# showlab/EgoVLP

Measured on AMD Instinct MI355X. Metric: clip-pairs/sec (whole node), 4f/224^2 ViT-B + 32-tok text, B=32/GPU, train step (fwd+gather+EgoNCE+bwd+AdamW), higher is better.
Workload: dtype fp16 (every Linear and both attentions of the video blocks, forward and backward) + bf16 (patch embedding, text tower, heads) MFMA operands, fp32 accumulate

## Files before the change

### egovlp_amd/csrc/gemm_nt.hip

```cpp
#include "common.h"
#include "egovlp_hip.h"

namespace {

constexpr int BM = 128, BN = 128, BK = 32;
constexpr int PLANE_BYTES = BM * BK * 2;

struct Frag4 {
  bf16x8_t v[4];
};

__device__ __forceinline__ int swz_g(int x) { return (0x78 >> (2 * x)) & 3; }

__device__ __forceinline__ void glds16(const void* g, char* lds_wave_base) {
  __builtin_amdgcn_global_load_lds((const __attribute__((address_space(1))) void*)g,
                                   (__attribute__((address_space(3))) void*)lds_wave_base, 16, 0, 0);
}

__device__ __forceinline__ void nt_epilogue4(const egv_gemm_desc& p, f32x4_t v, int m, int n) {
  if (p.alpha != 1.0f) v *= p.alpha;
  if (p.bias) v += *(const f32x4_t*)(p.bias + n);
  if (p.act == EGV_ACT_GELU) {
    if (p.aux_out) *(f32x4_t*)(p.aux_out + (long)m * p.ldaux + n) = v;
#pragma unroll
    for (int e = 0; e < 4; ++e) v[e] = gelu_f(v[e]);
  } else if (p.act == EGV_ACT_GELU_BWD) {
    const f32x4_t zv = *(const f32x4_t*)(p.aux_in + (long)m * p.ldaux + n);
#pragma unroll
    for (int e = 0; e < 4; ++e) v[e] *= gelu_grad_f(zv[e]);
  } else if (p.act == EGV_ACT_RELU_BWD) {
    const f32x4_t zv = *(const f32x4_t*)(p.aux_in + (long)m * p.ldaux + n);
#pragma unroll
    for (int e = 0; e < 4; ++e) v[e] = zv[e] > 0.f ? v[e] : 0.f;
  }
  if (p.residual) v += *(const f32x4_t*)(p.residual + (long)m * p.ldr + n);
  if (p.out_f32) *(f32x4_t*)(p.out_f32 + (long)m * p.ldo + n) = v;
  if (p.out_hi) {
    bf16_t h[4], l[4];
#pragma unroll
    for (int e = 0; e < 4; ++e) split_bf16(v[e], h[e], l[e]);
    *(u32x2_t*)(p.out_hi + (long)m * p.ldoh + n) = (u32x2_t){pack2(h[0], h[1]), pack2(h[2], h[3])};
    if (p.out_lo) *(u32x2_t*)(p.out_lo + (long)m * p.ldoh + n) = (u32x2_t){pack2(l[0], l[1]), pack2(l[2], l[3])};
  }
}

template <int PASSES>
__global__ __launch_bounds__(256, 2) void gemm_nt_kernel(const egv_gemm_desc p) {
  extern __shared__ __attribute__((aligned(16))) char smem[];
  constexpr int NPL = (PASSES == 3) ? 4 : 2;
  constexpr int STAGE_BYTES = NPL * PLANE_BYTES;

  const int tid = threadIdx.x;
  const int lane = tid & 63;
  const int wave = __builtin_amdgcn_readfirstlane(tid >> 6);
  const int wm = wave >> 1, wn = wave & 1;

  const int tiles_n = (p.N + BN - 1) / BN;
  const int tiles_m = (p.M + BM - 1) / BM;
  const int nwg = tiles_m * tiles_n;
  const int wg = xcd_remap(blockIdx.x, nwg);
  const int tm = wg / tiles_n, tn = wg % tiles_n;
  const int m0 = tm * BM, n0 = tn * BN;

  const int ksplit = p.ksplit > 1 ? p.ksplit : 1;
  const int z = blockIdx.y;
  const int ksteps_total = p.K / BK;
  const int ksteps_per = (ksteps_total + ksplit - 1) / ksplit;
  const int ks_begin = z * ksteps_per;
  const int ks_end = min(ksteps_total, ks_begin + ksteps_per);
  const int nk = ks_end - ks_begin;

  const int srcchunk = (lane & 3) ^ swz_g((lane >> 4) & 3);
  const bf16_t* asrc[2][2];
  const bf16_t* bsrc[2][2];
#pragma unroll
  for (int q = 0; q < 2; ++q) {
    const int row = (wave * 2 + q) * 16 + (lane >> 2);
    const long ar = min(m0 + row, p.M - 1);
    const long br = min(n0 + row, p.N - 1);
    const long koff = (long)ks_begin * BK + srcchunk * 8;
    asrc[0][q] = p.a_hi + ar * p.lda + koff;
    bsrc[0][q] = p.b_hi + br * p.ldb + koff;
    if (PASSES == 3) {
      asrc[1][q] = p.a_lo + ar * p.lda + koff;
      bsrc[1][q] = p.b_lo + br * p.ldb + koff;
    }
  }

  auto stage = [&](int buf) {
    char* base = smem + buf * STAGE_BYTES + wave * 2048;
#pragma unroll
    for (int q = 0; q < 2; ++q) {
      glds16(asrc[0][q], base + 0 * PLANE_BYTES + q * 1024);
      glds16(bsrc[0][q], base + (NPL / 2) * PLANE_BYTES + q * 1024);
      if (PASSES == 3) {
        glds16(asrc[1][q], base + 1 * PLANE_BYTES + q * 1024);
        glds16(bsrc[1][q], base + 3 * PLANE_BYTES + q * 1024);
      }
      asrc[0][q] += BK;
      bsrc[0][q] += BK;
      if (PASSES == 3) {
        asrc[1][q] += BK;
        bsrc[1][q] += BK;
      }
    }
  };

  const int frow = lane & 15;
  const int foff = frow * 64 + (((lane >> 4) ^ swz_g(frow >> 2)) * 16);
  const int a_off = (wm * 64) * 64 + foff;
  const int b_off = (wn * 64) * 64 + foff;

  f32x4_t acc[4][4];
#pragma unroll
  for (int i = 0; i < 4; ++i)
#pragma unroll
    for (int j = 0; j < 4; ++j) acc[i][j] = (f32x4_t){0.f, 0.f, 0.f, 0.f};

  if (nk > 0) stage(0);
  for (int t = 0; t < nk; ++t) {
    __syncthreads();
    if (t + 1 < nk) stage((t + 1) & 1);
    const char* sb = smem + (t & 1) * STAGE_BYTES;
    Frag4 ah, bh, al, bl;
#pragma unroll
    for (int f = 0; f < 4; ++f) {
      ah.v[f] = *(const bf16x8_t*)(sb + 0 * PLANE_BYTES + a_off + f * 16 * 64);
      bh.v[f] = *(const bf16x8_t*)(sb + (NPL / 2) * PLANE_BYTES + b_off + f * 16 * 64);
      if (PASSES == 3) {
        al.v[f] = *(const bf16x8_t*)(sb + 1 * PLANE_BYTES + a_off + f * 16 * 64);
        bl.v[f] = *(const bf16x8_t*)(sb + 3 * PLANE_BYTES + b_off + f * 16 * 64);
      }
    }
#pragma unroll
    for (int i = 0; i < 4; ++i)
#pragma unroll
      for (int j = 0; j < 4; ++j) {
        if (PASSES == 3) {
          acc[i][j] = __builtin_amdgcn_mfma_f32_16x16x32_bf16(bl.v[j], ah.v[i], acc[i][j], 0, 0, 0);
          acc[i][j] = __builtin_amdgcn_mfma_f32_16x16x32_bf16(bh.v[j], al.v[i], acc[i][j], 0, 0, 0);
        }
        acc[i][j] = __builtin_amdgcn_mfma_f32_16x16x32_bf16(bh.v[j], ah.v[i], acc[i][j], 0, 0, 0);
      }
  }

  const int lm = lane & 15;
  const int ln = (lane >> 4) * 4;
#pragma unroll
  for (int i = 0; i < 4; ++i) {
    const int m = m0 + wm * 64 + i * 16 + lm;
    if (m >= p.M) continue;
#pragma unroll
    for (int j = 0; j < 4; ++j) {
      const int n = n0 + wn * 64 + j * 16 + ln;
      if (n >= p.N) continue;
      f32x4_t v = acc[i][j];
      if (ksplit > 1) {
        *(f32x4_t*)(p.partial + ((long)z * p.M + m) * p.N + n) = v;
        continue;
      }
      nt_epilogue4(p, v, m, n);
    }
  }
}

__global__ __launch_bounds__(256) void splitk_reduce_kernel(const float* __restrict__ partial, float* __restrict__ out,
                                                            long mn, int ksplit, int accumulate,
                                                            const float* __restrict__ partial2, float* __restrict__ out2,
                                                            long n2, int blocks1) {
  if ((int)blockIdx.x >= blocks1) {
    partial = partial2;
    out = out2;
    mn = n2;
    accumulate = 0;
  }
  const long i4 = ((long)((int)blockIdx.x >= blocks1 ? (int)blockIdx.x - blocks1 : (int)blockIdx.x) * blockDim.x + threadIdx.x) * 4;
  if (i4 >= mn) return;
  f32x4_t s = egv_load<EGV_NT_REDUCE_LD, f32x4_t>(partial + i4);
  for (int z = 1; z < ksplit; ++z) s += egv_load<EGV_NT_REDUCE_LD, f32x4_t>(partial + (long)z * mn + i4);
  if (accumulate) s += *(const f32x4_t*)(out + i4);
  egv_store<EGV_NT_WGRAD>(out + i4, s);
}

constexpr int RED_MAX_T = 8;
struct ReduceTable {
  const float* partial[RED_MAX_T];
  float* out[RED_MAX_T];
  float* colsum[RED_MAX_T];
  long mn[RED_MAX_T];
  int m[RED_MAX_T], ks[RED_MAX_T];
  int blk_start[RED_MAX_T + 1];
  int blocks1[RED_MAX_T];
  int count;
};
__global__ __launch_bounds__(256) void splitk_reduce_multi_kernel(const ReduceTable t) {
  int e = 0;
  while (e + 1 < t.count && (int)blockIdx.x >= t.blk_start[e + 1]) ++e;
  const int local = (int)blockIdx.x - t.blk_start[e];
  const int ks = t.ks[e];
  const float* partial = t.partial[e];
  float* out = t.out[e];
  long mn = t.mn[e];
  long i4;
  if (local >= t.blocks1[e]) {
    partial += (long)ks * mn;
    out = t.colsum[e];
    mn = t.m[e];
    i4 = ((long)(local - t.blocks1[e]) * 256 + threadIdx.x) * 4;
  } else {
    i4 = ((long)local * 256 + threadIdx.x) * 4;
  }
  if (i4 >= mn) return;
  f32x4_t s = egv_load<EGV_NT_REDUCE_LD, f32x4_t>(partial + i4);
  for (int z = 1; z < ks; ++z) s += egv_load<EGV_NT_REDUCE_LD, f32x4_t>(partial + (long)z * mn + i4);
  egv_store<EGV_NT_WGRAD>(out + i4, s);
}

}

extern "C" int egv_splitk_reduce_multi(int32_t count, const float* const* partial, float* const* out, const int64_t* mn, const int32_t* ksplit,
                                       float* const* colsum, const int32_t* m, void* stream) {
  if (count < 1 || count > RED_MAX_T || !partial || !out || !mn || !ksplit) return EGV_ERR_ARG;
  ReduceTable t = {};
  int nb = 0;
  for (int i = 0; i < count; ++i) {
    if (!partial[i] || !out[i] || mn[i] <= 0 || mn[i] % 4 != 0 || ksplit[i] < 2) return EGV_ERR_ARG;
    const bool cs = colsum && colsum[i];
    if (cs && (!m || m[i] <= 0 || m[i] % 4 != 0)) return EGV_ERR_ARG;
    t.partial[i] = partial[i]; t.out[i] = out[i]; t.colsum[i] = cs ? colsum[i] : nullptr;
    t.mn[i] = mn[i]; t.m[i] = cs ? m[i] : 0; t.ks[i] = ksplit[i];
    t.blk_start[i] = nb;
    t.blocks1[i] = (int)((mn[i] / 4 + 255) / 256);
    nb += t.blocks1[i] + (cs ? (m[i] / 4 + 255) / 256 : 0);
  }
  t.blk_start[count] = nb;
  t.count = count;
  EGV_LAUNCH(splitk_reduce_multi_kernel, dim3(nb), dim3(256), 0, (hipStream_t)stream, t);
  EGV_CHECK_LAUNCH();
  return EGV_OK;
}

int egv_gemm_big_launch(const egv_gemm_desc& p, hipStream_t s, int variant);
bool egv_gemm_big_supports(const egv_gemm_desc& p);

__global__ __launch_bounds__(256) void splitk_reduce_epilogue_kernel(const egv_gemm_desc p, int ksplit) {
  const long i4 = ((long)blockIdx.x * blockDim.x + threadIdx.x) * 4;
  const long mn = (long)p.M * p.N;
  if (i4 >= mn) return;
  f32x4_t s = *(const f32x4_t*)(p.partial + i4);
  for (int z = 1; z < ksplit; ++z) s += *(const f32x4_t*)(p.partial + (long)z * mn + i4);
  const int m = (int)(i4 / p.N), n = (int)(i4 - (long)m * p.N);
  nt_epilogue4(p, s, m, n);
}

static int gemm_variant(const egv_gemm_desc& p) {
  const bool big_ok = egv_gemm_big_supports(p);
  if (p.trans) return big_ok ? 3 : -1;
  if (p.passes == 2 || p.passes == 4) return big_ok ? 3 : -1;
  const long big_tiles = (long)((p.M + 255) / 256) * ((p.N + 255) / 256) * (p.ksplit > 1 ? p.ksplit : 1);
  if (big_ok && big_tiles >= 128) return 3;
  return 1;
}

extern "C" int egv_gemm_nt(const egv_gemm_desc* d, void* stream) {
  const egv_gemm_desc& p = *d;
  if (!p.a_hi || !p.b_hi) return EGV_ERR_ARG;
  if (p.passes < 1 || p.passes > 4) return EGV_ERR_ARG;
  if ((p.passes == 2 || p.passes == 3) && (!p.a_lo || !p.b_lo)) return EGV_ERR_ARG;
  if (p.out_fmt < 0 || p.out_fmt > 4) return EGV_ERR_ARG;
  if (p.M <= 0 || p.N <= 0 || p.K <= 0) return EGV_ERR_ARG;
  if (p.N % 4 != 0 || p.lda % 8 != 0 || p.ldb % 8 != 0) return EGV_ERR_ARG;
  if (!p.trans && p.K % BK != 0) return EGV_ERR_ARG;
  if (p.ksplit > 1 && !p.partial) return EGV_ERR_ARG;
  if (p.colsum && !p.trans) return EGV_ERR_ARG;
  if (p.grid_cap != 0 && (p.grid_cap < 8 || p.grid_cap > 256 || p.grid_cap % 8 != 0)) return EGV_ERR_ARG;
  const int variant = gemm_variant(p);
  if (variant < 0) return EGV_ERR_ARG;
  if (p.aux_bf16 < 0 || p.aux_bf16 > 3) return EGV_ERR_ARG;
  if (p.aux_bf16 && (variant < 3 || p.act == EGV_ACT_RELU_BWD)) return EGV_ERR_ARG;
  if (p.aux_bf16 == 3 && p.passes != 4 && p.passes != 2) return EGV_ERR_ARG;
  if ((p.passes == 2 || p.passes == 4 || p.out_fmt != 0) && (variant < 3 || (p.passes != 2 && p.passes != 4))) return EGV_ERR_ARG;
  if ((p.passes == 2 || p.out_fmt != 0) && (p.trans || p.ksplit > 1)) return EGV_ERR_ARG;
  if (p.passes == 4 && !p.trans && p.ksplit > 1) return EGV_ERR_ARG;
  if (p.alpha != 1.0f && p.trans && !(p.alpha > 0.f)) return EGV_ERR_ARG;
  const int tiles = ((p.M + BM - 1) / BM) * ((p.N + BN - 1) / BN);
  const int ks = p.ksplit > 1 ? p.ksplit : 1;
  dim3 grid(tiles, ks), block(256);
  hipStream_t s = (hipStream_t)stream;
  if (variant >= 3) {
    const int rc = egv_gemm_big_launch(p, s, variant);
    if (rc) return rc;
  } else if (p.passes == 3) {
    EGV_LAUNCH(gemm_nt_kernel<3>, grid, block, 2 * 4 * PLANE_BYTES, s, p);
  } else {
    EGV_LAUNCH(gemm_nt_kernel<1>, grid, block, 2 * 2 * PLANE_BYTES, s, p);
  }
  EGV_CHECK_LAUNCH();
  if (ks > 1 && !p.trans && variant < 3) {
    if (p.accumulate) return EGV_ERR_ARG;
    const long mn4 = (long)p.M * p.N / 4;
    EGV_LAUNCH(splitk_reduce_epilogue_kernel, dim3((int)((mn4 + 255) / 256)), dim3(256), 0, s, p, ks);
    EGV_CHECK_LAUNCH();
  } else if (ks > 1 && p.accumulate == 2) {
    if (!p.trans || !p.out_f32 || p.ldo != p.N) return EGV_ERR_ARG;
  } else if (ks > 1) {
    if (!p.out_f32 || p.ldo != p.N) return EGV_ERR_ARG;
    const long mn = (long)p.M * p.N;
    const int blocks = (int)((mn / 4 + 255) / 256);
    if (p.colsum && p.M % 4 != 0) return EGV_ERR_ARG;
    const int blocks2 = p.colsum ? (p.M / 4 + 255) / 256 : 0;
    EGV_LAUNCH(splitk_reduce_kernel, dim3(blocks + blocks2), dim3(256), 0, s, p.partial, p.out_f32, mn, ks, p.accumulate,
               p.partial + (long)ks * mn, p.colsum, (long)p.M, blocks);
    EGV_CHECK_LAUNCH();
  }
  return EGV_OK;
}
```

### egovlp_amd/csrc/text_layer.hip

```cpp
#include <hip/hip_runtime.h>

#include "layer_call.h"

namespace {

bool geom_ok(const egv_text_geom& g) {
  if (g.B <= 0 || g.L <= 0 || g.H <= 0 || g.D != g.H * 64 || g.Hd <= 0 || g.D % 32 || g.Hd % 32) return false;
  if ((g.fwd_passes != 1 && g.fwd_passes != 3) || (g.bwd_passes != 1 && g.bwd_passes != 3) || g.bwd_passes > g.fwd_passes) return false;
  if (!(g.attn_p >= 0.0f && g.attn_p < 1.0f) || !(g.ffn_p >= 0.0f && g.ffn_p < 1.0f)) return false;
  for (int i = 0; i < 4; ++i)
    if (g.nt_ksplit_fwd[i] < 1 || g.nt_ksplit_bwd[i] < 1 || g.wgrad_ksplit[i] < 1) return false;
  return true;
}

void wshape(const egv_text_geom& g, int i, int64_t& N, int64_t& K) {
  switch (i) {
    case 0: N = 3 * (int64_t)g.D; K = g.D; break;
    case 1: N = g.D; K = g.D; break;
    case 2: N = g.Hd; K = g.D; break;
    default: N = g.D; K = g.Hd; break;
  }
}

struct FwdLayout {
  int64_t x_hi, x_lo, qkv, c_hi, c_lo, lse, s1, sa_hi, sa_lo, sa, mean1, rstd1, h_hi, h_lo, z, s2raw, s2, mean2, rstd2, partial;
  int64_t total;
};

FwdLayout fwd_layout(const egv_text_geom& g) {
  const int64_t M = (int64_t)g.B * g.L, D = g.D, Hd = g.Hd;
  const bool lo = g.fwd_passes == 3;
  FwdLayout L;
  Bump b;
  auto plane = [&](int64_t cols) { return b.take(M * cols * 2); };
  auto plane_lo = [&](int64_t cols) { return lo ? b.take(M * cols * 2) : (int64_t)-1; };
  L.x_hi = plane(D); L.x_lo = plane_lo(D);
  L.qkv = b.take(M * 3 * D * 4);
  L.c_hi = plane(D); L.c_lo = plane_lo(D);
  L.lse = b.take((int64_t)g.B * g.H * g.L * 4);
  L.s1 = b.take(M * D * 4);
  L.sa_hi = plane(D); L.sa_lo = plane_lo(D);
  L.sa = b.take(M * D * 4);
  L.mean1 = b.take(M * 4); L.rstd1 = b.take(M * 4);
  L.h_hi = plane(Hd); L.h_lo = plane_lo(Hd);
  L.z = g.train ? b.take(M * Hd * 4) : (int64_t)-1;
  L.s2raw = g.ffn_p > 0.0f ? b.take(M * D * 4) : (int64_t)-1;
  L.s2 = b.take(M * D * 4);
  L.mean2 = b.take(M * 4); L.rstd2 = b.take(M * 4);
  int64_t pmax = 0;
  for (int i = 0; i < 4; ++i) {
    int64_t N, K;
    wshape(g, i, N, K);
    if (g.nt_ksplit_fwd[i] > 1) pmax = pmax > g.nt_ksplit_fwd[i] * M * N * 4 ? pmax : g.nt_ksplit_fwd[i] * M * N * 4;
  }
  L.partial = pmax ? b.take(pmax) : (int64_t)-1;
  L.total = b.off;
  return L;
}

struct BwdLayout {
  int64_t d_s2, g_in, g_hi, g_lo, dz_hi, dz_lo, d_sa, d_s1, ds1_hi, ds1_lo, d_ctx, dqkv, dqkv_hi, dqkv_lo, ln_work, attn_work, partial;
  int64_t total;
};

int64_t bwd_nt_cols(const egv_text_geom& g, int i) { return i == 0 ? g.Hd : g.D; }

BwdLayout bwd_layout(const egv_text_geom& g) {
  const int64_t M = (int64_t)g.B * g.L, D = g.D, Hd = g.Hd;
  const bool lo = g.bwd_passes == 3;
  BwdLayout L;
  Bump b;
  auto plane = [&](int64_t cols) { return b.take(M * cols * 2); };
  auto plane_lo = [&](int64_t cols) { return lo ? b.take(M * cols * 2) : (int64_t)-1; };
  L.d_s2 = b.take(M * D * 4);
  L.g_in = g.ffn_p > 0.0f ? b.take(M * D * 4) : (int64_t)-1;
  L.g_hi = plane(D); L.g_lo = plane_lo(D);
  L.dz_hi = plane(Hd); L.dz_lo = plane_lo(Hd);
  L.d_sa = b.take(M * D * 4);
  L.d_s1 = b.take(M * D * 4);
  L.ds1_hi = plane(D); L.ds1_lo = plane_lo(D);
  L.d_ctx = b.take(M * D * 4);
  L.dqkv = b.take(M * 3 * D * 4);
  L.dqkv_hi = plane(3 * D); L.dqkv_lo = plane_lo(3 * D);
  L.ln_work = b.take(2 * D * (int64_t)egv_layernorm_bwd_parts((int32_t)M) * 4);
  L.attn_work = b.take((int64_t)g.B * g.H * g.L * 4);
  int64_t pmax = 0;
  for (int i = 0; i < 4; ++i) {
    if (g.nt_ksplit_bwd[i] > 1) {
      const int64_t by = g.nt_ksplit_bwd[i] * M * bwd_nt_cols(g, i) * 4;
      pmax = pmax > by ? pmax : by;
    }
    int64_t N, K;
    wshape(g, i, N, K);
    if (g.wgrad_ksplit[i] > 1) {
      const int64_t by = (int64_t)g.wgrad_ksplit[i] * (N * K + N) * 4;
      pmax = pmax > by ? pmax : by;
    }
  }
  L.partial = pmax ? b.take(pmax) : (int64_t)-1;
  L.total = b.off;
  return L;
}

void grad_layout(const egv_text_geom& g, int64_t off[12], int64_t& total) {
  int64_t p = 0;
  auto take = [&](int64_t n) { const int64_t q = p; p += n; return q; };
  for (int i = 0; i < 4; ++i) { int64_t N, K; wshape(g, i, N, K); off[i] = take(N * K); }
  for (int i = 0; i < 4; ++i) { int64_t N, K; wshape(g, i, N, K); off[4 + i] = take(N); }
  for (int i = 0; i < 4; ++i) off[8 + i] = take(g.D);
  total = p;
}

}

extern "C" int64_t egv_text_layer_fwd_arena_bytes(const egv_text_geom* g) { return (g && geom_ok(*g)) ? fwd_layout(*g).total : -1; }
extern "C" int64_t egv_text_layer_bwd_arena_bytes(const egv_text_geom* g) { return (g && geom_ok(*g)) ? bwd_layout(*g).total : -1; }

extern "C" int egv_text_layer_grad_layout(const egv_text_geom* g, int64_t* offsets12, int64_t* total_floats) {
  if (!g || !geom_ok(*g) || !offsets12 || !total_floats) return EGV_ERR_ARG;
  grad_layout(*g, offsets12, *total_floats);
  return EGV_OK;
}

extern "C" int egv_text_layer_fwd(const egv_text_geom* gp, const egv_text_params* pp, const float* x, const int64_t* mask, float* out,
                                  void* arena, void* stream) {
  if (!gp || !pp || !x || !mask || !out || !arena || !geom_ok(*gp)) return EGV_ERR_ARG;
  const egv_text_geom& g = *gp;
  const egv_text_params& p = *pp;
  const FwdLayout L = fwd_layout(g);
  const int P = g.fwd_passes;
  const int32_t M = g.B * g.L, D = g.D, Hd = g.Hd;
  for (int i = 0; i < 4; ++i)
    if (!p.w_hi[i] || (P == 3 && !p.w_lo[i])) return EGV_ERR_ARG;
  char* A = (char*)arena;
  egv_bf16 *x_hi = at<egv_bf16>(A, L.x_hi), *x_lo = at<egv_bf16>(A, L.x_lo);
  egv_bf16 *c_hi = at<egv_bf16>(A, L.c_hi), *c_lo = at<egv_bf16>(A, L.c_lo);
  egv_bf16 *sa_hi = at<egv_bf16>(A, L.sa_hi), *sa_lo = at<egv_bf16>(A, L.sa_lo);
  egv_bf16 *h_hi = at<egv_bf16>(A, L.h_hi), *h_lo = at<egv_bf16>(A, L.h_lo);
  float *qkv = at<float>(A, L.qkv), *s1 = at<float>(A, L.s1), *sa = at<float>(A, L.sa), *s2 = at<float>(A, L.s2);
  float* part = at<float>(A, L.partial);

  EGV_TRY(egv_split_f32(x, D, M, D, x_hi, x_lo, D, nullptr, nullptr, 0, nullptr, stream));
  {
    egv_gemm_desc d = nt_desc(x_hi, x_lo, D, p.w_hi[0], p.w_lo[0], p.ldw[0], M, 3 * D, D, P, g.grid_cap, g.nt_ksplit_fwd[0], part);
    d.bias = p.bias[0]; d.out_f32 = qkv; d.ldo = 3 * D;
    EGV_TRY(egv_gemm_nt(&d, stream));
  }
  EGV_TRY(egv_text_attn_fwd(qkv, qkv + D, qkv + 2 * D, 3 * D, mask, g.B, g.L, g.H, P, g.attn_p, g.attn_seed, g.seed_dev, c_hi, c_lo,
                            at<float>(A, L.lse), stream));
  {
    egv_gemm_desc d = nt_desc(c_hi, c_lo, D, p.w_hi[1], p.w_lo[1], p.ldw[1], M, D, D, P, g.grid_cap, g.nt_ksplit_fwd[1], part);
    d.bias = p.bias[1]; d.residual = x; d.ldr = D; d.out_f32 = s1; d.ldo = D;
    EGV_TRY(egv_gemm_nt(&d, stream));
  }
  EGV_TRY(egv_layernorm_fwd(s1, nullptr, D, p.ln1w, p.ln1b, g.eps, M, D, nullptr, sa_hi, sa_lo, sa, D, at<float>(A, L.mean1),
                            at<float>(A, L.rstd1), stream));
  {
    egv_gemm_desc d = nt_desc(sa_hi, sa_lo, D, p.w_hi[2], p.w_lo[2], p.ldw[2], M, Hd, D, P, g.grid_cap, g.nt_ksplit_fwd[2], part);
    d.bias = p.bias[2]; d.act = EGV_ACT_GELU; d.out_hi = h_hi; d.out_lo = h_lo; d.ldoh = Hd;
    if (g.train) { d.aux_out = at<float>(A, L.z); d.ldaux = Hd; }
    EGV_TRY(egv_gemm_nt(&d, stream));
  }
  {
    egv_gemm_desc d = nt_desc(h_hi, h_lo, Hd, p.w_hi[3], p.w_lo[3], p.ldw[3], M, D, Hd, P, g.grid_cap, g.nt_ksplit_fwd[3], part);
    d.bias = p.bias[3];
    if (g.ffn_p > 0.0f) {
      float* raw = at<float>(A, L.s2raw);
      d.out_f32 = raw; d.ldo = D;
      EGV_TRY(egv_gemm_nt(&d, stream));
      EGV_TRY(egv_dropout(raw, sa, s2, (int64_t)M * D, g.ffn_p, g.ffn_seed, g.seed_dev, stream));
    } else {
      d.residual = sa; d.ldr = D; d.out_f32 = s2; d.ldo = D;
      EGV_TRY(egv_gemm_nt(&d, stream));
    }
  }
  return egv_layernorm_fwd(s2, nullptr, D, p.ln2w, p.ln2b, g.eps, M, D, nullptr, nullptr, nullptr, out, D, at<float>(A, L.mean2),
                           at<float>(A, L.rstd2), stream);
}

extern "C" int egv_text_layer_bwd(const egv_text_geom* gp, const egv_text_params* pp, const float* g_out, const int64_t* mask,
                                  const void* fwd_arena, void* bwd_arena, float* d_x, float* grads, void* stream) {
  if (!gp || !pp || !g_out || !mask || !fwd_arena || !bwd_arena || !d_x || !grads || !geom_ok(*gp) || !gp->train) return EGV_ERR_ARG;
  const egv_text_geom& g = *gp;
  const egv_text_params& p = *pp;
  const FwdLayout F = fwd_layout(g);
  const BwdLayout L = bwd_layout(g);
  int64_t goff[12], gtot;
  grad_layout(g, goff, gtot);
  const int Pb = g.bwd_passes;
  const int32_t M = g.B * g.L, D = g.D, Hd = g.Hd;
  for (int i = 0; i < 4; ++i)
    if (!p.wt_hi[i] || (Pb == 3 && !p.wt_lo[i])) return EGV_ERR_ARG;
  const char* FA = (const char*)fwd_arena;
  char* A = (char*)bwd_arena;
  const egv_bf16 *x_hi, *x_lo, *c_hi, *c_lo, *sa_hi, *sa_lo, *h_hi, *h_lo;
  saved_planes(FA, Pb, F.x_hi, F.x_lo, x_hi, x_lo);
  saved_planes(FA, Pb, F.c_hi, F.c_lo, c_hi, c_lo);
  saved_planes(FA, Pb, F.sa_hi, F.sa_lo, sa_hi, sa_lo);
  saved_planes(FA, Pb, F.h_hi, F.h_lo, h_hi, h_lo);
  const float *qkv = at<float>(FA, F.qkv), *s1 = at<float>(FA, F.s1), *s2 = at<float>(FA, F.s2);
  float* part = at<float>(A, L.partial);
  float* ln_work = at<float>(A, L.ln_work);

  auto wgrad = [&](int i, const egv_bf16* dy_hi, const egv_bf16* dy_lo, int64_t lddy, const egv_bf16* a_hi, const egv_bf16* a_lo,
                   int64_t lda) -> int {
    int64_t N, K;
    wshape(g, i, N, K);
    const egv_gemm_desc d = tn_desc(dy_hi, dy_lo, lddy, a_hi, a_lo, lda, N, K, M, Pb, grads + goff[i], grads + goff[4 + i], g.wgrad_ksplit[i],
                                    part, g.grid_cap);
    return egv_gemm_nt(&d, stream);
  };

  float* d_s2 = at<float>(A, L.d_s2);
  EGV_TRY(egv_layernorm_bwd(g_out, nullptr, nullptr, D, s2, D, p.ln2w, at<float>(FA, F.mean2), at<float>(FA, F.rstd2), M, D, nullptr, nullptr,
                            d_s2, D, nullptr, nullptr, grads + goff[10], grads + goff[11], ln_work, stream));
  const float* g_in = d_s2;
  if (g.ffn_p > 0.0f) {
    float* gi = at<float>(A, L.g_in);
    EGV_TRY(egv_dropout(d_s2, nullptr, gi, (int64_t)M * D, g.ffn_p, g.ffn_seed, g.seed_dev, stream));
    g_in = gi;
  }
  egv_bf16 *g_hi = at<egv_bf16>(A, L.g_hi), *g_lo = at<egv_bf16>(A, L.g_lo);
  EGV_TRY(egv_split_f32(g_in, D, M, D, g_hi, g_lo, D, nullptr, nullptr, 0, nullptr, stream));
  egv_bf16 *dz_hi = at<egv_bf16>(A, L.dz_hi), *dz_lo = at<egv_bf16>(A, L.dz_lo);
  {
    egv_gemm_desc d = nt_desc(g_hi, g_lo, D, p.wt_hi[3], p.wt_lo[3], p.ldwt[3], M, Hd, D, Pb, g.grid_cap, g.nt_ksplit_bwd[0], part);
    d.act = EGV_ACT_GELU_BWD; d.aux_in = at<float>(FA, F.z); d.ldaux = Hd;
    d.out_hi = dz_hi; d.out_lo = dz_lo; d.ldoh = Hd;
    EGV_TRY(egv_gemm_nt(&d, stream));
  }
  EGV_TRY(wgrad(3, g_hi, g_lo, D, h_hi, h_lo, Hd));
  EGV_TRY(wgrad(2, dz_hi, dz_lo, Hd, sa_hi, sa_lo, D));
  float* d_sa = at<float>(A, L.d_sa);
  {
    egv_gemm_desc d = nt_desc(dz_hi, dz_lo, Hd, p.wt_hi[2], p.wt_lo[2], p.ldwt[2], M, D, Hd, Pb, g.grid_cap, g.nt_ksplit_bwd[1], part);
    d.residual = d_s2; d.ldr = D; d.out_f32 = d_sa; d.ldo = D;
    EGV_TRY(egv_gemm_nt(&d, stream));
  }
  float* d_s1 = at<float>(A, L.d_s1);
  EGV_TRY(egv_layernorm_bwd(d_sa, nullptr, nullptr, D, s1, D, p.ln1w, at<float>(FA, F.mean1), at<float>(FA, F.rstd1), M, D, nullptr, nullptr,
                            d_s1, D, nullptr, nullptr, grads + goff[8], grads + goff[9], ln_work, stream));
  egv_bf16 *ds1_hi = at<egv_bf16>(A, L.ds1_hi), *ds1_lo = at<egv_bf16>(A, L.ds1_lo);
  EGV_TRY(egv_split_f32(d_s1, D, M, D, ds1_hi, ds1_lo, D, nullptr, nullptr, 0, nullptr, stream));
  EGV_TRY(wgrad(1, ds1_hi, ds1_lo, D, c_hi, c_lo, D));
  float* d_ctx = at<float>(A, L.d_ctx);
  {
    egv_gemm_desc d = nt_desc(ds1_hi, ds1_lo, D, p.wt_hi[1], p.wt_lo[1], p.ldwt[1], M, D, D, Pb, g.grid_cap, g.nt_ksplit_bwd[2], part);
    d.out_f32 = d_ctx; d.ldo = D;
    EGV_TRY(egv_gemm_nt(&d, stream));
  }
  float* dqkv = at<float>(A, L.dqkv);
  EGV_TRY(egv_text_attn_bwd(qkv, qkv + D, qkv + 2 * D, 3 * D, mask, d_ctx, at<float>(FA, F.lse), g.B, g.L, g.H, Pb, g.attn_p, g.attn_seed,
                            g.seed_dev, dqkv, dqkv + D, dqkv + 2 * D, 3 * D, at<float>(A, L.attn_work), stream));
  egv_bf16 *dq_hi = at<egv_bf16>(A, L.dqkv_hi), *dq_lo = at<egv_bf16>(A, L.dqkv_lo);
  EGV_TRY(egv_split_f32(dqkv, 3 * D, M, 3 * D, dq_hi, dq_lo, 3 * D, nullptr, nullptr, 0, nullptr, stream));
  EGV_TRY(wgrad(0, dq_hi, dq_lo, 3 * D, x_hi, x_lo, D));
  {
    egv_gemm_desc d = nt_desc(dq_hi, dq_lo, 3 * D, p.wt_hi[0], p.wt_lo[0], p.ldwt[0], M, D, 3 * D, Pb, g.grid_cap, g.nt_ksplit_bwd[3], part);
    d.residual = d_s1; d.ldr = D; d.out_f32 = d_x; d.ldo = D;
    EGV_TRY(egv_gemm_nt(&d, stream));
  }
  return EGV_OK;
}
```

Before: 1014.

## Add multi-stage LDS ring pipeline for small GEMMs and fuse text-bwd splits into layernorm

Adds a new small-tile NT GEMM kernel that uses a 4-stage LDS ring with direct global-to-LDS loads, fine-grained vmcnt waits and double-buffered register fragments. It is enabled by default through an environment toggle and replaces the two-stage kernel used by non-big GEMMs, aiming to hide global load latency. The text-layer backward also has the layernorm-backward write the bf16 hi/lo splits directly, which removes separate split kernels. Behind a compile flag, it can batch the split-k weight-gradient reductions into one multi-reduce launch. The deeper ring uses much more LDS per block (launch bounds allow 2 blocks), which may lower occupancy.

```diff
diff --git a/egovlp_amd/csrc/gemm_nt.hip b/egovlp_amd/csrc/gemm_nt.hip
--- a/egovlp_amd/csrc/gemm_nt.hip
+++ b/egovlp_amd/csrc/gemm_nt.hip
@@ -1,3 +1,5 @@
+#include <type_traits>
+
 #include "common.h"
 #include "egovlp_hip.h"
 
@@ -5,6 +7,7 @@
 
 constexpr int BM = 128, BN = 128, BK = 32;
 constexpr int PLANE_BYTES = BM * BK * 2;
+constexpr int RING_STAGES = 4;
 
 struct Frag4 {
   bf16x8_t v[4];
@@ -143,6 +146,181 @@
         acc[i][j] = __builtin_amdgcn_mfma_f32_16x16x32_bf16(bh.v[j], ah.v[i], acc[i][j], 0, 0, 0);
       }
   }
+
+  const int lm = lane & 15;
+  const int ln = (lane >> 4) * 4;
+#pragma unroll
+  for (int i = 0; i < 4; ++i) {
+    const int m = m0 + wm * 64 + i * 16 + lm;
+    if (m >= p.M) continue;
+#pragma unroll
+    for (int j = 0; j < 4; ++j) {
+      const int n = n0 + wn * 64 + j * 16 + ln;
+      if (n >= p.N) continue;
+      f32x4_t v = acc[i][j];
+      if (ksplit > 1) {
+        *(f32x4_t*)(p.partial + ((long)z * p.M + m) * p.N + n) = v;
+        continue;
+      }
+      nt_epilogue4(p, v, m, n);
+    }
+  }
+}
+
+template <int N>
+__device__ __forceinline__ void ring_wait() {
+  static_assert(N >= 0 && N < 64, "vmcnt is a 6-bit count");
+  asm volatile("" ::: "memory");
+  __builtin_amdgcn_s_waitcnt((N & 15) | ((N >> 4) << 14) | (7 << 4));
+  asm volatile("" ::: "memory");
+}
+template <int NI, int MAXC>
+__device__ __forceinline__ void ring_wait_tiles(int c) {
+  if constexpr (MAXC <= 0) {
+    ring_wait<0>();
+  } else {
+    if (c >= MAXC) ring_wait<NI * MAXC>();
+    else ring_wait_tiles<NI, MAXC - 1>(c);
+  }
+}
+
+template <int PASSES, int S>
+__global__ __launch_bounds__(256, 2) void gemm_nt_ring_kernel(const egv_gemm_desc p) {
+  extern __shared__ __attribute__((aligned(16))) char smem[];
+  constexpr int NPL = (PASSES == 3) ? 4 : 2;
+  constexpr int STAGE_BYTES = NPL * PLANE_BYTES;
+  constexpr int NI = 2 * NPL;
+  static_assert(S >= 3 && S <= 5 && S * STAGE_BYTES <= 160 * 1024 && NI * (S - 2) < 64, "ring depth");
+
+  const int tid = threadIdx.x;
+  const int lane = tid & 63;
+  const int wave = __builtin_amdgcn_readfirstlane(tid >> 6);
+  const int wm = wave >> 1, wn = wave & 1;
+
+  const int tiles_n = (p.N + BN - 1) / BN;
+  const int tiles_m = (p.M + BM - 1) / BM;
+  const int nwg = tiles_m * tiles_n;
+  const int wg = xcd_remap(blockIdx.x, nwg);
+  const int tm = wg / tiles_n, tn = wg % tiles_n;
+  const int m0 = tm * BM, n0 = tn * BN;
+
+  const int ksplit = p.ksplit > 1 ? p.ksplit : 1;
+  const int z = blockIdx.y;
+  const int ksteps_total = p.K / BK;
+  const int ksteps_per = (ksteps_total + ksplit - 1) / ksplit;
+  const int ks_begin = z * ksteps_per;
+  const int ks_end = min(ksteps_total, ks_begin + ksteps_per);
+  const int nk = __builtin_amdgcn_readfirstlane(max(ks_end - ks_begin, 0));
+
+  const int srcchunk = (lane & 3) ^ swz_g((lane >> 4) & 3);
+  const bf16_t* asrc[2];
+  const bf16_t* bsrc[2];
+  const long a_lo_d = PASSES == 3 ? p.a_lo - p.a_hi : 0, b_lo_d = PASSES == 3 ? p.b_lo - p.b_hi : 0;
+#pragma unroll
+  for (int q = 0; q < 2; ++q) {
+    const int row = (wave * 2 + q) * 16 + (lane >> 2);
+    const long ar = min(m0 + row, p.M - 1);
+    const long br = min(n0 + row, p.N - 1);
+    const long koff = (long)ks_begin * BK + srcchunk * 8;
+    asrc[q] = p.a_hi + ar * p.lda + koff;
+    bsrc[q] = p.b_hi + br * p.ldb + koff;
+  }
+
+  auto stage = [&](int buf) {
+    char* base = smem + buf * STAGE_BYTES + wave * 2048;
+#pragma unroll
+    for (int q = 0; q < 2; ++q) {
+      glds16(asrc[q], base + 0 * PLANE_BYTES + q * 1024);
+      glds16(bsrc[q], base + (NPL / 2) * PLANE_BYTES + q * 1024);
+      if (PASSES == 3) {
+        glds16(asrc[q] + a_lo_d, base + 1 * PLANE_BYTES + q * 1024);
+        glds16(bsrc[q] + b_lo_d, base + 3 * PLANE_BYTES + q * 1024);
+      }
+      asrc[q] += BK;
+      bsrc[q] += BK;
+    }
+  };
+
+  const int frow = lane & 15;
+  const int foff = frow * 64 + (((lane >> 4) ^ swz_g(frow >> 2)) * 16);
+  const int a_off = (wm * 64) * 64 + foff;
+  const int b_off = (wn * 64) * 64 + foff;
+
+  struct Frags {
+    Frag4 ah, bh, al, bl;
+  };
+  auto read_frags = [&](Frags& f, int buf) {
+    const char* sb = smem + buf * STAGE_BYTES;
+#pragma unroll
+    for (int i = 0; i < 4; ++i) {
+      f.ah.v[i] = *(const bf16x8_t*)(sb + 0 * PLANE_BYTES + a_off + i * 16 * 64);
+      f.bh.v[i] = *(const bf16x8_t*)(sb + (NPL / 2) * PLANE_BYTES + b_off + i * 16 * 64);
+      if (PASSES == 3) {
+        f.al.v[i] = *(const bf16x8_t*)(sb + 1 * PLANE_BYTES + a_off + i * 16 * 64);
+        f.bl.v[i] = *(const bf16x8_t*)(sb + 3 * PLANE_BYTES + b_off + i * 16 * 64);
+      }
+    }
+  };
+
+  f32x4_t acc[4][4];
+#pragma unroll
+  for (int i = 0; i < 4; ++i)
+#pragma unroll
+    for (int j = 0; j < 4; ++j) acc[i][j] = (f32x4_t){0.f, 0.f, 0.f, 0.f};
+
+  auto multiply = [&](const Frags& f) {
+#pragma unroll
+    for (int i = 0; i < 4; ++i)
+#pragma unroll
+      for (int j = 0; j < 4; ++j) {
+        if (PASSES == 3) {
+          acc[i][j] = __builtin_amdgcn_mfma_f32_16x16x32_bf16(f.bl.v[j], f.ah.v[i], acc[i][j], 0, 0, 0);
+          acc[i][j] = __builtin_amdgcn_mfma_f32_16x16x32_bf16(f.bh.v[j], f.al.v[i], acc[i][j], 0, 0, 0);
+        }
+        acc[i][j] = __builtin_amdgcn_mfma_f32_16x16x32_bf16(f.bh.v[j], f.ah.v[i], acc[i][j], 0, 0, 0);
+      }
+  };
+
+  int rd = 0, wr = S - 1;
+  auto next_stage = [](int b) { return b + 1 == S ? 0 : b + 1; };
+  auto kstep = [&](auto steady, int t, const Frags& cur, Frags& nxt) {
+    constexpr bool STEADY = decltype(steady)::value;
+    if constexpr (STEADY) ring_wait<NI * (S - 3)>();
+    else ring_wait_tiles<NI, S - 3>(nk - 2 - t);
+    __builtin_amdgcn_s_barrier();
+    if (STEADY || t + S - 1 < nk) stage(wr);
+    wr = next_stage(wr);
+    read_frags(nxt, rd);
+    rd = next_stage(rd);
+    __builtin_amdgcn_sched_barrier(0);
+    multiply(cur);
+    __builtin_amdgcn_sched_barrier(0);
+  };
+
+  Frags f0, f1;
+  if (nk > 0) {
+#pragma unroll
+    for (int s = 0; s < S - 1; ++s)
+      if (s < nk) stage(s);
+    ring_wait_tiles<NI, S - 2>(nk - 1);
+    __builtin_amdgcn_s_barrier();
+    read_frags(f0, rd);
+    rd = next_stage(rd);
+  }
+  int t = 0;
+  for (; t + 1 + S <= nk; t += 2) {
+    kstep(std::true_type{}, t, f0, f1);
+    kstep(std::true_type{}, t + 1, f1, f0);
+  }
+  for (; t + 2 < nk; t += 2) {
+    kstep(std::false_type{}, t, f0, f1);
+    kstep(std::false_type{}, t + 1, f1, f0);
+  }
+  if (nk - t == 2) {
+    kstep(std::false_type{}, t, f0, f1);
+    f0 = f1;
+  }
+  if (nk > 0) multiply(f0);
 
   const int lm = lane & 15;
   const int ln = (lane >> 4) * 4;
@@ -260,6 +438,28 @@
   const long big_tiles = (long)((p.M + 255) / 256) * ((p.N + 255) / 256) * (p.ksplit > 1 ? p.ksplit : 1);
   if (big_ok && big_tiles >= 128) return 3;
   return 1;
+}
+
+static bool small_gemm_ring() {
+  static const bool v = [] {
+    const char* e = getenv("EGV_SMALL_GEMM_RING");
+    return !e || atoi(e) != 0;
+  }();
+  return v;
+}
+
+template <int PASSES>
+static int launch_ring(const egv_gemm_desc& p, dim3 grid, hipStream_t s) {
+  constexpr int lds = RING_STAGES * (PASSES == 3 ? 4 : 2) * PLANE_BYTES;
+  auto k = gemm_nt_ring_kernel<PASSES, RING_STAGES>;
+  static bool attr_set = false;
+  if (!attr_set) {
+    if (hipFuncSetAttribute((const void*)k, hipFuncAttributeMaxDynamicSharedMemorySize, lds) != hipSuccess)
+      return EGV_ERR_LAUNCH + (int)hipGetLastError();
+    attr_set = true;
+  }
+  EGV_LAUNCH(k, grid, dim3(256), lds, s, p);
+  return EGV_OK;
 }
 
 extern "C" int egv_gemm_nt(const egv_gemm_desc* d, void* stream) {
@@ -290,6 +490,9 @@
   if (variant >= 3) {
     const int rc = egv_gemm_big_launch(p, s, variant);
     if (rc) return rc;
+  } else if (small_gemm_ring()) {
+    const int rc = p.passes == 3 ? launch_ring<3>(p, grid, s) : launch_ring<1>(p, grid, s);
+    if (rc) return rc;
   } else if (p.passes == 3) {
     EGV_LAUNCH(gemm_nt_kernel<3>, grid, block, 2 * 4 * PLANE_BYTES, s, p);
   } else {
diff --git a/egovlp_amd/csrc/text_layer.hip b/egovlp_amd/csrc/text_layer.hip
--- a/egovlp_amd/csrc/text_layer.hip
+++ b/egovlp_amd/csrc/text_layer.hip
@@ -60,6 +60,7 @@
 
 struct BwdLayout {
   int64_t d_s2, g_in, g_hi, g_lo, dz_hi, dz_lo, d_sa, d_s1, ds1_hi, ds1_lo, d_ctx, dqkv, dqkv_hi, dqkv_lo, ln_work, attn_work, partial;
+  int64_t wpartial[4];
   int64_t total;
 };
 
@@ -90,14 +91,25 @@
       const int64_t by = g.nt_ksplit_bwd[i] * M * bwd_nt_cols(g, i) * 4;
       pmax = pmax > by ? pmax : by;
     }
+#ifndef EGV_TEXT_MULTI_REDUCE
     int64_t N, K;
     wshape(g, i, N, K);
     if (g.wgrad_ksplit[i] > 1) {
       const int64_t by = (int64_t)g.wgrad_ksplit[i] * (N * K + N) * 4;
       pmax = pmax > by ? pmax : by;
     }
+#endif
   }
   L.partial = pmax ? b.take(pmax) : (int64_t)-1;
+  for (int i = 0; i < 4; ++i) {
+#ifdef EGV_TEXT_MULTI_REDUCE
+    int64_t N, K;
+    wshape(g, i, N, K);
+    L.wpartial[i] = g.wgrad_ksplit[i] > 1 ? b.take((int64_t)g.wgrad_ksplit[i] * (N * K + N) * 4) : (int64_t)-1;
+#else
+    L.wpartial[i] = g.wgrad_ksplit[i] > 1 ? L.partial : (int64_t)-1;
+#endif
+  }
   L.total = b.off;
   return L;
 }
@@ -206,22 +218,24 @@
                    int64_t lda) -> int {
     int64_t N, K;
     wshape(g, i, N, K);
-    const egv_gemm_desc d = tn_desc(dy_hi, dy_lo, lddy, a_hi, a_lo, lda, N, K, M, Pb, grads + goff[i], grads + goff[4 + i], g.wgrad_ksplit[i],
-                                    part, g.grid_cap);
+    egv_gemm_desc d = tn_desc(dy_hi, dy_lo, lddy, a_hi, a_lo, lda, N, K, M, Pb, grads + goff[i], grads + goff[4 + i], g.wgrad_ksplit[i],
+                              at<float>(A, L.wpartial[i]), g.grid_cap);
+#ifdef EGV_TEXT_MULTI_REDUCE
+    if (d.ksplit > 1) d.accumulate = 2;
+#endif
     return egv_gemm_nt(&d, stream);
   };
 
   float* d_s2 = at<float>(A, L.d_s2);
+  egv_bf16 *g_hi = at<egv_bf16>(A, L.g_hi), *g_lo = at<egv_bf16>(A, L.g_lo);
+  const bool drop = g.ffn_p > 0.0f;
   EGV_TRY(egv_layernorm_bwd(g_out, nullptr, nullptr, D, s2, D, p.ln2w, at<float>(FA, F.mean2), at<float>(FA, F.rstd2), M, D, nullptr, nullptr,
-                            d_s2, D, nullptr, nullptr, grads + goff[10], grads + goff[11], ln_work, stream));
-  const float* g_in = d_s2;
-  if (g.ffn_p > 0.0f) {
+                            d_s2, D, drop ? nullptr : g_hi, drop ? nullptr : g_lo, grads + goff[10], grads + goff[11], ln_work, stream));
+  if (drop) {
     float* gi = at<float>(A, L.g_in);
     EGV_TRY(egv_dropout(d_s2, nullptr, gi, (int64_t)M * D, g.ffn_p, g.ffn_seed, g.seed_dev, stream));
-    g_in = gi;
-  }
-  egv_bf16 *g_hi = at<egv_bf16>(A, L.g_hi), *g_lo = at<egv_bf16>(A, L.g_lo);
-  EGV_TRY(egv_split_f32(g_in, D, M, D, g_hi, g_lo, D, nullptr, nullptr, 0, nullptr, stream));
+    EGV_TRY(egv_split_f32(gi, D, M, D, g_hi, g_lo, D, nullptr, nullptr, 0, nullptr, stream));
+  }
   egv_bf16 *dz_hi = at<egv_bf16>(A, L.dz_hi), *dz_lo = at<egv_bf16>(A, L.dz_lo);
   {
     egv_gemm_desc d = nt_desc(g_hi, g_lo, D, p.wt_hi[3], p.wt_lo[3], p.ldwt[3], M, Hd, D, Pb, g.grid_cap, g.nt_ksplit_bwd[0], part);
@@ -238,10 +252,9 @@
     EGV_TRY(egv_gemm_nt(&d, stream));
   }
   float* d_s1 = at<float>(A, L.d_s1);
+  egv_bf16 *ds1_hi = at<egv_bf16>(A, L.ds1_hi), *ds1_lo = at<egv_bf16>(A, L.ds1_lo);
   EGV_TRY(egv_layernorm_bwd(d_sa, nullptr, nullptr, D, s1, D, p.ln1w, at<float>(FA, F.mean1), at<float>(FA, F.rstd1), M, D, nullptr, nullptr,
-                            d_s1, D, nullptr, nullptr, grads + goff[8], grads + goff[9], ln_work, stream));
-  egv_bf16 *ds1_hi = at<egv_bf16>(A, L.ds1_hi), *ds1_lo = at<egv_bf16>(A, L.ds1_lo);
-  EGV_TRY(egv_split_f32(d_s1, D, M, D, ds1_hi, ds1_lo, D, nullptr, nullptr, 0, nullptr, stream));
+                            d_s1, D, ds1_hi, ds1_lo, grads + goff[8], grads + goff[9], ln_work, stream));
   EGV_TRY(wgrad(1, ds1_hi, ds1_lo, D, c_hi, c_lo, D));
   float* d_ctx = at<float>(A, L.d_ctx);
   {
@@ -260,5 +273,24 @@
     d.residual = d_s1; d.ldr = D; d.out_f32 = d_x; d.ldo = D;
     EGV_TRY(egv_gemm_nt(&d, stream));
   }
+  {
+    const float* wp[4];
+    float *outp[4], *csp[4];
+    int64_t mn[4];
+    int32_t ksv[4], mv[4];
+    int cnt = 0;
+    for (int i = 0; i < 4; ++i) {
+      if (g.wgrad_ksplit[i] <= 1) continue;
+      int64_t N, K;
+      wshape(g, i, N, K);
+      wp[cnt] = at<float>(A, L.wpartial[i]); outp[cnt] = grads + goff[i]; csp[cnt] = grads + goff[4 + i];
+      mn[cnt] = N * K; ksv[cnt] = g.wgrad_ksplit[i]; mv[cnt] = (int32_t)N;
+      ++cnt;
+    }
+#ifndef EGV_TEXT_MULTI_REDUCE
+    cnt = 0;
+#endif
+    if (cnt) EGV_TRY(egv_splitk_reduce_multi(cnt, wp, outp, mn, ksv, csp, mv, stream));
+  }
   return EGV_OK;
 }
```

Measured after the change: 1013. Within noise of the previous version (-0.1%).
